# liupei101/AdvMIL

Measured on AMD Instinct MI355X. Metric: WSI bags/sec (full G+D step), higher is better.
Workload: dtype bf16x3 (fp32 operands split hi+lo, 3 bf16 MFMAs per product, fp32 accumulate; fp32 storage); 1 GPU; ABMIL+AdvMIL(RLIP prj discriminator), 8192-patch x 1024 fp32 bags (BASELINE.json configs[1] shape; fp32 storage, bf16x3 split arithmetic: >= the bf16 the config names, within 2e-5 of the fp32 reference); gen_updates=1, distinct_resident_bags_per_gpu=64, parallelism=bag-parallel dp1, dropout=shipped rates, launch=hipGraph replay (4 captured bag groups)

## Files before the change

### advmil_amd/_lib.py

```python
import ctypes
import os
from ctypes import c_float, c_int, c_int32, c_int64, c_size_t, c_uint64, c_void_p

LIB_PATH = os.environ.get("ADVMIL_HIP_LIB") or os.path.join(os.path.dirname(os.path.abspath(__file__)), "libadvmil_hip.so")


class HipLibraryMissing(RuntimeError):
    pass


class AdvmilHipError(RuntimeError):
    pass


class Epilogue(ctypes.Structure):
    _fields_ = [("bias", c_void_p), ("act0", c_int), ("act1", c_int), ("act_split", c_int), ("drop_p", c_float),
                ("seed", c_void_p), ("stream_id", c_uint64), ("rowv", c_void_p), ("colv", c_void_p), ("rowseg", c_void_p),
                ("maskref", c_void_p), ("ldmask", c_int), ("mask_scale", c_float), ("accumulate", c_int),
                ("alpha", c_float), ("a_hi", c_void_p), ("a_lo", c_void_p), ("b_hi", c_void_p), ("b_lo", c_void_p),
                ("c_hi", c_void_p), ("c_lo", c_void_p), ("gate_wc", c_void_p), ("gate_out", c_void_p), ("gate_np", c_int),
                ("rng_row", c_void_p), ("c2", c_void_p), ("ldc2", c_int64), ("n_split", c_int64), ("bias2", c_void_p), ("colsum", c_void_p), ("maskbits", c_void_p), ("ldbits", c_int64),
                ("gate_bits_a", c_void_p), ("gate_bits_b", c_void_p), ("ldgbits", c_int64), ("c_rows_pair32", c_int)]


# ... 35 lines not shown
                ("step", c_void_p), ("la_state", c_void_p), ("m_sched", c_void_p), ("p_hi", c_void_p), ("p_lo", c_void_p),
                ("abs_partial", c_void_p), ("clear_grad", ctypes.c_int32)]


OPT_KINDS = {"adam": 0, "adamw": 1, "nadam": 2, "radam": 3, "adadelta": 4}


SIGNATURES = {
    "advmil_version": (c_int, []),
    "advmil_gemm_f32_workspace_bytes": (c_size_t, [c_int64, c_int64, c_int]),
    "advmil_gemm_f32": (c_int, [c_int, c_int, c_int64, c_int64, c_int64, c_void_p, c_int64, c_void_p, c_int64, c_void_p,
                                c_int64, ctypes.POINTER(Epilogue), c_int, c_void_p, c_size_t, c_void_p]),
    "advmil_split_planes": (c_int, [c_void_p, c_int64, c_void_p, c_void_p, c_void_p]),
    "advmil_stage_bag": (c_int, [c_void_p, c_void_p, c_size_t, c_void_p, c_void_p, c_void_p, c_void_p, c_size_t, c_void_p]),
    "advmil_gate_interleave": (c_int, [c_void_p, c_void_p, c_void_p, c_void_p, c_int, c_void_p, c_void_p, c_void_p, c_void_p, c_int, c_void_p]),
    "advmil_gate_partial_sum": (c_int, [c_void_p, c_int, c_void_p, c_int64, c_void_p, c_void_p]),
    "advmil_gemm_f32_gate_blocks": (c_int, [c_int, c_int64]),
    "advmil_gemm_f32_colsum_rows": (c_int64, [c_int, c_int64, c_int64]),
    "advmil_merge_partials": (c_int, [c_void_p, c_int, c_int64, c_int64, c_void_p, c_int, c_void_p]),
    "advmil_set_gemm_mode": (c_int, [c_int]),
    "advmil_get_gemm_mode": (c_int, []),
    "advmil_gemm_f32_plan": (c_int, [c_int64, c_int64, c_int64, ctypes.POINTER(c_int), ctypes.POINTER(c_int)]),
    "advmil_gemm_f32_plan_layout": (c_int, [c_int, c_int, c_int64, c_int64, c_int64, ctypes.POINTER(c_int), ctypes.POINTER(c_int)]),
    "advmil_gemm_f32_plan_planes": (c_int, [c_int, c_int, c_int64, c_int64, c_int64, ctypes.POINTER(c_int)]),
    "advmil_gemm_f32_plan_tn_planes": (c_int, [c_int64, c_int64, c_int64, ctypes.POINTER(c_int), ctypes.POINTER(c_int)]),
    "advmil_gemm_f32_tiled": (c_int, [c_int, c_int, c_int64, c_int64, c_int64, c_void_p, c_int64, c_void_p, c_int64, c_void_p,
                                      c_int64, ctypes.POINTER(Epilogue), c_int, c_int, c_void_p, c_size_t, c_void_p]),
    "advmil_mha_fwd": (c_int, [c_void_p, c_void_p, c_int64, c_int, c_int, c_int, c_void_p, c_int64, c_float, c_void_p, c_uint64,
                               c_void_p, c_void_p, c_void_p, c_void_p]),
    "advmil_mha_fwd_lse": (c_int, [c_void_p, c_void_p, c_int64, c_int, c_int, c_int, c_void_p, c_int64, c_float, c_void_p, c_uint64,
# ... 10 lines not shown
    "advmil_add_dropout_ln_bwd": (c_int, [c_void_p, c_void_p, c_void_p, c_void_p, c_void_p, c_int64, c_int64, c_float, c_void_p,
                                          c_uint64, c_void_p, c_void_p, c_void_p, c_void_p, c_void_p, c_int, c_void_p, c_size_t,
                                          c_void_p]),
    "advmil_gate_score_fwd": (c_int, [c_void_p, c_void_p, c_void_p, c_float, c_void_p, c_uint64, c_uint64, c_int64, c_int64,
                                      c_void_p, c_void_p, c_void_p]),
    "advmil_softmax_pool_workspace_bytes": (c_size_t, [c_int64, c_int64, c_int]),
    "advmil_softmax_pool_fwd": (c_int, [c_void_p, c_void_p, c_int64, c_int64, c_int64, c_int, c_void_p, c_int64, c_void_p,
                                        c_void_p, c_void_p, c_size_t, c_void_p]),
    "advmil_softmax_pool_mean_workspace_bytes": (c_size_t, [c_int64, c_int64, c_int]),
    "advmil_softmax_pool_mean_fwd": (c_int, [c_void_p, c_void_p, c_int64, c_int64, c_int64, c_int, c_void_p, c_int64, c_void_p,
                                             c_void_p, c_void_p, c_void_p, c_size_t, c_void_p]),
    "advmil_softmax_pool_bwd": (c_int, [c_void_p, c_void_p, c_void_p, c_void_p, c_int64, c_int64, c_int64, c_int, c_void_p,
                                        c_int64, c_void_p, c_void_p, c_size_t, c_void_p]),
    "advmil_softmax_pool_fwd_planes": (c_int, [c_void_p, c_void_p, c_void_p, c_int64, c_int64, c_int64, c_int, c_void_p, c_int64, c_void_p,
                                               c_void_p, c_void_p, c_size_t, c_void_p]),
    "advmil_softmax_pool_bwd_planes": (c_int, [c_void_p, c_void_p, c_void_p, c_void_p, c_void_p, c_int64, c_int64, c_int64, c_int, c_void_p,
                                               c_int64, c_void_p, c_void_p, c_size_t, c_void_p]),
    "advmil_dropout_planes": (c_int, [c_void_p, c_void_p, c_int64, c_int64, c_float, c_void_p, c_uint64, c_void_p, c_void_p, c_void_p, c_void_p,
                                      c_float, c_uint64, c_uint64, c_void_p, c_void_p, c_void_p]),
    "advmil_gate_bwd_workspace_bytes": (c_size_t, [c_int64, c_int64]),
    "advmil_gate_bwd": (c_int, [c_void_p, c_void_p, c_void_p, c_float, c_void_p, c_uint64, c_uint64, c_int64, c_int64,
                                c_void_p, c_void_p, c_void_p, c_void_p, c_int, c_void_p, c_void_p, c_void_p, c_int, c_void_p, c_size_t,
                                c_void_p]),
    "advmil_colsum_workspace_bytes": (c_size_t, [c_int64, c_int64]),
    "advmil_act_dropout_bwd": (c_int, [c_void_p, c_void_p, c_int, c_float, c_void_p, c_uint64, c_int64, c_int64, c_void_p,
                                       c_void_p, c_int, c_void_p, c_void_p, c_void_p, c_void_p, c_void_p, c_size_t, c_void_p]),
    "advmil_colsum": (c_int, [c_void_p, c_int64, c_int64, c_void_p, c_int, c_void_p, c_size_t, c_void_p]),
    "advmil_ln_relu_mean16_fwd": (c_int, [c_void_p, c_void_p, c_void_p, c_float, c_int64, c_int64, c_void_p, c_void_p,
                                          c_void_p, c_void_p, c_void_p, c_int, c_void_p]),
    "advmil_ln_relu_mean16_bwd_workspace_bytes": (c_size_t, [c_int64, c_int64]),
# ... 102 lines not shown
```

### advmil_amd/csrc/pool.hip

```cpp
#include <cstdlib>
#include "common.h"
#include "bf16split.h"
#include "sumq.h"
#include "../../include/advmil_hip.h"

#define ROWS_PER_BLOCK 32
static inline int rows_per_block(int64_t rows) {
  int64_t r = (rows + 1023) / 1024;
  r = (r + 31) / 32 * 32;
  if (r < ROWS_PER_BLOCK) r = ROWS_PER_BLOCK;
  if (r > 512) r = 512;
  return (int)r;
}

struct RowColMap {
  int cols4, rpp, c4, r;
  bool active;
};
__device__ __forceinline__ RowColMap make_map(int64_t D) {
  RowColMap m;
  m.cols4 = (int)(D >> 2);
  m.rpp = 256 / m.cols4;
  if (m.rpp < 1) m.rpp = 1;
  m.c4 = threadIdx.x % m.cols4;
// ... 279 lines not shown
}

__device__ __forceinline__ void planes8(const bf16raw* __restrict__ hi, const bf16raw* __restrict__ lo, int64_t off, float4& v0, float4& v1) {
  const uint4 a = *reinterpret_cast<const uint4*>(hi + off);
  const uint4 b = *reinterpret_cast<const uint4*>(lo + off);
  v0.x = __uint_as_float(a.x << 16) + __uint_as_float(b.x << 16);
  v0.y = __uint_as_float(a.x & 0xffff0000u) + __uint_as_float(b.x & 0xffff0000u);
  v0.z = __uint_as_float(a.y << 16) + __uint_as_float(b.y << 16);
  v0.w = __uint_as_float(a.y & 0xffff0000u) + __uint_as_float(b.y & 0xffff0000u);
  v1.x = __uint_as_float(a.z << 16) + __uint_as_float(b.z << 16);
  v1.y = __uint_as_float(a.z & 0xffff0000u) + __uint_as_float(b.z & 0xffff0000u);
  v1.z = __uint_as_float(a.w << 16) + __uint_as_float(b.w << 16);
  v1.w = __uint_as_float(a.w & 0xffff0000u) + __uint_as_float(b.w & 0xffff0000u);
}

template <bool MEAN, bool PL = false>
__global__ __launch_bounds__(256) void pool_partial8_online_kernel(const float* __restrict__ s, const float* __restrict__ h, int64_t ldh,
                                                                   int64_t N, int64_t D, const int64_t* __restrict__ seg_ptr,
                                                                   float* __restrict__ partial, float* __restrict__ pstats, int rpb,
                                                                   float* __restrict__ mpartial, const bf16raw* __restrict__ hlo = nullptr) {
  __shared__ __attribute__((aligned(16))) float red[2048];
  __shared__ float wts[512];
  __shared__ float wred[8];
  const int cols8 = (int)(D >> 3), rpp = 256 / cols8;
  const int c8 = threadIdx.x % cols8, rl = threadIdx.x / cols8;
  const int tid = threadIdx.x, lane = tid & 63, w = tid >> 6;
  const int b = blockIdx.y;
  int64_t beg, end;
  seg_range(seg_ptr, b, N, beg, end);
  const int64_t r0 = beg + (int64_t)blockIdx.x * rpb;
  float* pst = pstats + ((int64_t)b * gridDim.x + blockIdx.x) * 2;
  float* prow = partial + ((int64_t)b * gridDim.x + blockIdx.x) * D;
  float* mrow = MEAN ? mpartial + ((int64_t)b * gridDim.x + blockIdx.x) * D : nullptr;
  if (r0 >= end) {
    if (tid < (int)(D >> 2)) {
      *reinterpret_cast<float4*>(prow + tid * 4) = make_float4(0.f, 0.f, 0.f, 0.f);
      if (MEAN) *reinterpret_cast<float4*>(mrow + tid * 4) = make_float4(0.f, 0.f, 0.f, 0.f);
    }
    if (tid == 0) { pst[0] = -INFINITY; pst[1] = 0.f; }
    return;
  }
  float mx = -INFINITY;
  for (int r = tid; r < rpb; r += 256) {
    const int64_t n = r0 + r;
    const float v = n < end ? s[n] : -INFINITY;
    wts[r] = v;
    mx = fmaxf(mx, v);
  }
  mx = wave_max(mx);
  if (lane == 0) wred[w] = mx;
  __syncthreads();
  mx = fmaxf(fmaxf(wred[0], wred[1]), fmaxf(wred[2], wred[3]));
  float ls = 0.f;
  for (int r = tid; r < rpb; r += 256) {
    const float e = (r0 + r < end) ? hw_exp(wts[r] - mx) : 0.f;
    wts[r] = e;
    ls += e;
  }
  ls = wave_sum(ls);
  if (lane == 0) wred[4 + w] = ls;
// ... 130 lines not shown
  }
  for (int64_t n = beg + (int64_t)blockIdx.x * 256 + tid; n < end; n += (int64_t)gridDim.x * 256) A[n] = hw_exp(s[n] - M) * inv;
}

static inline int64_t pool_nblk(int64_t max_len) { const int r = rows_per_block(max_len); return (max_len + r - 1) / r; }

extern "C" size_t advmil_softmax_pool_workspace_bytes(int64_t max_len, int64_t D, int nseg) {
  if (nseg < 1) nseg = 1;
  const int64_t a = 4 * (int64_t)nseg + (int64_t)nseg * pool_nblk(max_len) * (D + 2);
  const int64_t b = 4 + (int64_t)nseg * ((max_len + 3) / 4);
  return (size_t)(a > b ? a : b) * sizeof(float);
}

static int softmax_pool_fwd_impl(const float* s, const float* h, int64_t ldh, int64_t N, int64_t D, int nseg, const int64_t* seg_ptr,
                                 int64_t max_len, float* A, float* pooled, float* mean, void* ws, size_t ws_bytes, hipStream_t stream,
                                 const bf16raw* hlo = nullptr);

extern "C" int advmil_softmax_pool_fwd(const float* s, const float* h, int64_t ldh, int64_t N, int64_t D, int nseg,
                                       const int64_t* seg_ptr, int64_t max_len, float* A, float* pooled, void* ws,
                                       size_t ws_bytes, advmil_stream_t stream_) {
  return softmax_pool_fwd_impl(s, h, ldh, N, D, nseg, seg_ptr, max_len, A, pooled, nullptr, ws, ws_bytes, (hipStream_t)stream_);
}

extern "C" int advmil_softmax_pool_fwd_planes(const float* s, const void* h_hi, const void* h_lo, int64_t ldh, int64_t N, int64_t D, int nseg,
                                              const int64_t* seg_ptr, int64_t max_len, float* A, float* pooled, void* ws,
                                              size_t ws_bytes, advmil_stream_t stream_) {
  if (!h_hi || !h_lo) return ADVMIL_EINVAL;
  return softmax_pool_fwd_impl(s, (const float*)h_hi, ldh, N, D, nseg, seg_ptr, max_len, A, pooled, nullptr, ws, ws_bytes, (hipStream_t)stream_,
                               (const bf16raw*)h_lo);
}

static inline size_t pool_mean_offset_bytes(int64_t max_len, int64_t D, int nseg) {
  return (advmil_softmax_pool_workspace_bytes(max_len, D, nseg) + 15) / 16 * 16;
}

extern "C" size_t advmil_softmax_pool_mean_workspace_bytes(int64_t max_len, int64_t D, int nseg) {
  if (nseg < 1) nseg = 1;
  return pool_mean_offset_bytes(max_len, D, nseg) + (size_t)((int64_t)nseg * pool_nblk(max_len) * D) * sizeof(float);
}

extern "C" int advmil_softmax_pool_mean_fwd(const float* s, const float* h, int64_t ldh, int64_t N, int64_t D, int nseg,
                                            const int64_t* seg_ptr, int64_t max_len, float* A, float* pooled, float* mean, void* ws,
                                            size_t ws_bytes, advmil_stream_t stream_) {
  if (!mean) return ADVMIL_EINVAL;
  return softmax_pool_fwd_impl(s, h, ldh, N, D, nseg, seg_ptr, max_len, A, pooled, mean, ws, ws_bytes, (hipStream_t)stream_);
}

static int softmax_pool_fwd_impl(const float* s, const float* h, int64_t ldh, int64_t N, int64_t D, int nseg, const int64_t* seg_ptr,
                                 int64_t max_len, float* A, float* pooled, float* mean, void* ws, size_t ws_bytes, hipStream_t stream,
                                 const bf16raw* hlo) {
  if (!s || !h || !A || !pooled || !ws || N <= 0 || D <= 0 || (D & 3) || D > 1024 || (ldh & 3)) return ADVMIL_EINVAL;
  if (ldh < D || ((uintptr_t)h & 15)) return ADVMIL_EINVAL;
  if (hlo && (((uintptr_t)hlo & 15) || (D & 7) || (ldh & 7) || D < 16 || mean)) return ADVMIL_EINVAL;
  if (!seg_ptr && nseg > 1) return ADVMIL_EINVAL;
  if (!seg_ptr) { nseg = 1; max_len = N; }
  if (nseg < 1 || max_len <= 0 || max_len > N) return ADVMIL_EINVAL;
  if (ws_bytes < (mean ? advmil_softmax_pool_mean_workspace_bytes(max_len, D, nseg) : advmil_softmax_pool_workspace_bytes(max_len, D, nseg)))
    return ADVMIL_EWORKSPACE;
  float* stats = (float*)ws;
  float* partial = stats + 4 * nseg;
  const int nblk = (int)pool_nblk(max_len);
  if ((D & 7) == 0 && D >= 16 && nblk <= POOL_ONLINE_MAX_NBLK) {
    float* pstats = partial + (int64_t)nseg * nblk * D;
    if (mean) {
      float* mpartial = (float*)ws + pool_mean_offset_bytes(max_len, D, nseg) / sizeof(float);
      hipLaunchKernelGGL((pool_partial8_online_kernel<true, false>), dim3(nblk, nseg), dim3(256), 0, stream, s, h, ldh, N, D, seg_ptr, partial, pstats,
                         rows_per_block(max_len), mpartial, (const bf16raw*)nullptr);
      ADVMIL_LAUNCH_CHECK();
      hipLaunchKernelGGL(pool_merge_online_kernel, dim3((unsigned)((D + 15) / 16), nseg), dim3(256), 0, stream, partial, pstats, nblk, D, s,
                         N, seg_ptr, pooled, A, stats, (const float*)mpartial, mean);
      ADVMIL_LAUNCH_CHECK();
      return ADVMIL_OK;
    }
    if (hlo)
      hipLaunchKernelGGL((pool_partial8_online_kernel<false, true>), dim3(nblk, nseg), dim3(256), 0, stream, s, h, ldh, N, D, seg_ptr, partial,
                         pstats, rows_per_block(max_len), (float*)nullptr, hlo);
    else
      hipLaunchKernelGGL((pool_partial8_online_kernel<false, false>), dim3(nblk, nseg), dim3(256), 0, stream, s, h, ldh, N, D, seg_ptr, partial,
                         pstats, rows_per_block(max_len), (float*)nullptr, (const bf16raw*)nullptr);
    ADVMIL_LAUNCH_CHECK();
    hipLaunchKernelGGL(pool_merge_online_kernel, dim3((unsigned)((D + 15) / 16), nseg), dim3(256), 0, stream, partial, pstats, nblk, D, s,
                       N, seg_ptr, pooled, A, stats, (const float*)nullptr, (float*)nullptr);
    ADVMIL_LAUNCH_CHECK();
    return ADVMIL_OK;
  }
  if (mean || hlo) return ADVMIL_EINVAL;
  hipLaunchKernelGGL(softmax_stats_kernel, dim3(nseg), dim3(1024), 0, stream, s, N, seg_ptr, stats);
  ADVMIL_LAUNCH_CHECK();
  if ((D & 7) == 0 && D >= 16)
    hipLaunchKernelGGL(pool_partial8_kernel, dim3(nblk, nseg), dim3(256), 0, stream, s, h, ldh, N, D, seg_ptr, stats, A, partial,
                       rows_per_block(max_len));
  else
    hipLaunchKernelGGL(pool_partial_kernel, dim3(nblk, nseg), dim3(256), 0, stream, s, h, ldh, N, D, seg_ptr, stats, A, partial,
                       rows_per_block(max_len));
  ADVMIL_LAUNCH_CHECK();
  hipLaunchKernelGGL(colsum_merge_kernel, dim3((unsigned)((D + 15) / 16), nseg), dim3(256), 0, stream, partial, nblk, D, D, pooled,
                     0, (int64_t)nblk * D, D);
  ADVMIL_LAUNCH_CHECK();
  return ADVMIL_OK;
}

// ... 232 lines not shown
  for (int64_t n = (int64_t)blockIdx.x * 256 + threadIdx.x; n < N; n += (int64_t)gridDim.x * 256) {
    float a = 0.f;
    for (int j = 0; j < np; ++j) a += partial[n * np + j];
    s[n] = a + b;
  }
}
extern "C" int advmil_gate_interleave(const float* Wa, const float* Wb, const float* ba, const float* bb, int D, float* Wi, void* Wi_hi,
                                      void* Wi_lo, float* bi, int pair32, advmil_stream_t stream_) {
  if (!Wa || !Wb || !ba || !bb || !Wi || !bi || D <= 0 || (D & 3) || ((Wi_hi != nullptr) != (Wi_lo != nullptr))) return ADVMIL_EINVAL;
  if (pair32 && (D & 31)) return ADVMIL_EINVAL;
  if (((uintptr_t)Wa & 15) || ((uintptr_t)Wb & 15) || ((uintptr_t)Wi & 15) || ((uintptr_t)Wi_hi & 7) || ((uintptr_t)Wi_lo & 7)) return ADVMIL_EINVAL;
  int64_t blocks = ((int64_t)2 * D * (D >> 2) + 255) / 256;
  if (blocks > 1024) blocks = 1024;
  hipLaunchKernelGGL(gate_interleave_kernel, dim3((unsigned)blocks), dim3(256), 0, (hipStream_t)stream_, Wa, Wb, ba, bb, D, Wi,
                     (bf16raw*)Wi_hi, (bf16raw*)Wi_lo, bi, pair32);
  ADVMIL_LAUNCH_CHECK();
  return ADVMIL_OK;
}
extern "C" int advmil_gate_partial_sum(const float* partial, int np, const float* bc, int64_t N, float* s, advmil_stream_t stream_) {
  if (!partial || !s || np <= 0 || N <= 0) return ADVMIL_EINVAL;
  int64_t blocks = (N + 255) / 256;
  if (blocks > 2048) blocks = 2048;
  hipLaunchKernelGGL(gate_partial_sum_kernel, dim3((unsigned)blocks), dim3(256), 0, (hipStream_t)stream_, partial, np, bc, N, s);
  ADVMIL_LAUNCH_CHECK();
  return ADVMIL_OK;
}

__global__ __launch_bounds__(256) void gate_bwd_kernel(const float* __restrict__ ab, const float* __restrict__ ds,
                                                       const float* __restrict__ wc, float p, const uint64_t* seed,
                                                       uint64_t stream_a, uint64_t stream_b, int64_t N, int64_t D,
// ... 839 lines not shown
```

### advmil_amd/ops.py

```python
import ctypes
import os

import torch

from . import _lib
from ._lib import Epilogue

ACT_NONE, ACT_RELU, ACT_TANH, ACT_SIGMOID = 0, 1, 2, 3
FUSED_WGRAD = True
KERNEL_PROFILE = None
STAMPS = None


class Stamps:

    def __init__(self, device, cap=2048):
        self.buf = torch.zeros(cap, dtype=torch.int64, device=device)
        self.tags = []
        self.khz = int(_lib.lib().advmil_clock_rate_khz()) or 100000

    def mark(self, tag):
        i = len(self.tags)
        if i >= self.buf.numel():
            return
# ... 296 lines not shown
        return Planes(torch.empty_strided(x.shape, x.stride(), dtype=torch.bfloat16, device=x.device),
                      torch.empty_strided(x.shape, x.stride(), dtype=torch.bfloat16, device=x.device))

    def view_rows(self, r0, r1):
        return Planes(self.hi[r0:r1], None if self.lo is None else self.lo[r0:r1])


USE_PLANES = os.environ.get("ADVMIL_PLANES", "1") != "0"
DH_NT_FUSED = os.environ.get("ADVMIL_DH_NT_FUSED", "1") != "0"
ACT_BWD_IN_DH = os.environ.get("ADVMIL_ACT_BWD_IN_DH", "1") != "0"
DG_PLANES_ONLY = os.environ.get("ADVMIL_DG_PLANES_ONLY", "1") != "0"
DW_PLANES = os.environ.get("ADVMIL_DW_PLANES", "1") != "0"
MEMO_PLANES = os.environ.get("ADVMIL_MEMO_PLANES", "1") != "0"
H_PLANES_ONLY = os.environ.get("ADVMIL_H_PLANES_ONLY", "1") != "0"
FUSED_GATE_TRAIN = os.environ.get("ADVMIL_FUSED_GATE_TRAIN", "1") != "0"
SLAB_PLANES_ANY = os.environ.get("ADVMIL_SLAB_PLANES_ANY", "1") != "0"
GENERIC_PLANES = os.environ.get("ADVMIL_GENERIC_PLANES", "1") != "0"
SMALL_LINEAR = os.environ.get("ADVMIL_SMALL_LINEAR", "1") != "0"
SMALL_LINEAR_ROWS = int(os.environ.get("ADVMIL_SMALL_LINEAR_ROWS", "8"))


def slab_takes_planes(rows, C):
    return bool(rows >= 4096 and USE_PLANES and get_gemm_mode() == "bf16x3" and (SLAB_PLANES_ANY or gemm_plan_planes(rows, 128, C)))


def planes_transposed(pl):
    R, C = pl.hi.shape
    out = Planes.alloc((C, R), pl.hi.device)
    d = (pl.lo.data_ptr() - pl.hi.data_ptr()) // 2
    do = (out.lo.data_ptr() - out.hi.data_ptr()) // 2
# ... 320 lines not shown
            self._div[k] = Segments([v // k for v in self.lens], self.device)
        return self._div[k]

    def twice(self):
        if "x2" not in self._div:
            self._div["x2"] = Segments(self.lens + self.lens, self.device)
        return self._div["x2"]

    def uniform(self, rows):
        key = ("u", rows)
        if key not in self._div:
            self._div[key] = Segments([rows] * self.nseg, self.device)
        return self._div[key]


def softmax_pool(s, h, N, D, seg=None, hpl=None):
    L = _lib.lib()
    nseg = 1 if seg is None else seg.nseg
    mlen = N if seg is None else seg.max_len
    A = torch.empty(N, dtype=torch.float32, device=h.device)
    pooled = torch.empty(nseg, D, dtype=torch.float32, device=h.device)
    wsb = L.advmil_softmax_pool_workspace_bytes(mlen, D, nseg)
    ws = _ws(wsb, h.device)
    big = STAMPS is not None and N * D >= (1 << 24)
    if big:
        _stamp("b", "softmax_pool_fwd", (N, D, nseg), 4.0 * N * D + 12.0 * N)
    if hpl is not None:
        _lib.check(L.advmil_softmax_pool_fwd_planes(_p(s), _p(hpl.hi), _p(hpl.lo), hpl.hi.stride(0), N, D, nseg,
                                                    _p(None if seg is None else seg.ptr), mlen, _p(A), _p(pooled), _p(ws), wsb, _stream()),
                   "softmax_pool_fwd_planes")
    else:
        _lib.check(L.advmil_softmax_pool_fwd(_p(s), _p(h), h.stride(0), N, D, nseg, _p(None if seg is None else seg.ptr), mlen, _p(A),
                                             _p(pooled), _p(ws), wsb, _stream()), "softmax_pool_fwd")
    if big:
        _stamp("e", "softmax_pool_fwd", (N, D, nseg), 4.0 * N * D + 12.0 * N)
    return A, pooled


def softmax_pool_mean(s, h, N, D, seg=None):
    L = _lib.lib()
    nseg = 1 if seg is None else seg.nseg
    mlen = N if seg is None else seg.max_len
    A = torch.empty(N, dtype=torch.float32, device=h.device)
    pooled = torch.empty(nseg, D, dtype=torch.float32, device=h.device)
    mean = torch.empty(nseg, D, dtype=torch.float32, device=h.device)
    wsb = L.advmil_softmax_pool_mean_workspace_bytes(mlen, D, nseg)
    ws = _ws(wsb, h.device)
    _lib.check(L.advmil_softmax_pool_mean_fwd(_p(s), _p(h), h.stride(0), N, D, nseg, _p(None if seg is None else seg.ptr), mlen, _p(A),
                                              _p(pooled), _p(mean), _p(ws), wsb, _stream()), "softmax_pool_mean_fwd")
    return A, pooled, mean

# ... 384 lines not shown
            if xpl is None and is_bf16_slab(x):
                x = as_f32(x)
            if ctx.gW is not None:
                gemm(dpre, x, False, False, N, K, M, out=ctx.gW.view(N, K), ldc=K, accumulate=True, b_planes=xpl)
            else:
                dW = gemm(dpre, x, False, False, N, K, M, b_planes=xpl).reshape(wshape)
        dx = gemm(dpre, W2, True, False, M, K, N) if need_x else None
        return dx, dW, (None if ctx.gb is not None else db), None, None, None, None, None, None, None, None, None


class ForwardMemo:

    def __init__(self):
        self.mode, self.token, self.rows_ptr, self.store = None, None, None, {}
        self.derived, self.ln = {}, {}

    def begin(self, mode, token, rows):
        if token != self.token:
            self.store.clear(); self.derived.clear(); self.ln.clear()
        self.mode, self.token, self.rows_ptr = mode, token, rows.data_ptr()

    def knows(self, x):
        return self.mode is not None and (x.data_ptr() == self.rows_ptr or (MEMO_CHAIN and x.data_ptr() in self.derived))

    def end(self, clear=False):
        self.mode = None
        if clear:
            self.store.clear(); self.derived.clear(); self.ln.clear()


MEMO = ForwardMemo()
MEMO_CHAIN = os.environ.get("ADVMIL_MEMO_CHAIN", "1") != "0"
MEMO_MIN_ROWS = int(os.environ.get("ADVMIL_MEMO_MIN_ROWS", "4096"))


PREFILL = {}
TWO_LAYERS = os.environ.get("ADVMIL_TWO_LAYERS", "1") != "0"


def prefill_two_layers(X, layer1, layer2):
    (W1, b1, a1, emit1), (W2, b2, a2, _) = layer1, layer2
    if not TWO_LAYERS or X.dim() != 2 or not X.is_contiguous():
        return False
# ... 101 lines not shown


class GatedAttnPoolFn(torch.autograd.Function):

    @staticmethod
    def forward(ctx, h, Wa, ba, Wb, bb, wc, bc, p, seed, sa, sb, seg, nograd=False, rr=None, hpl=None, act_fuse=None, gate=None):
        _chk(h, "h")
        h = h.contiguous()
        N, D = h.shape
        ctx.act_fuse = act_fuse
        ctx.pair32 = False
        wcv = wc.detach().reshape(-1)
        stale = hpl is not None and hpl.fp32_stale
        ppl = hpl if stale else None
        if FUSED_GATE_SCORE and p <= 0.0 and N >= 4096 and nograd:
            Wi, bi, wipl = gate_interleave(Wa.detach(), ba.detach(), Wb.detach(), bb.detach(), D, planes=hpl is not None)
            s = gate_partial_sum(gemm(h, Wi, True, True, N, 2 * D, D, bias=bi, gate_wc=wcv, a_planes=hpl, b_planes=wipl), bc.detach())
            A, pooled = softmax_pool(s, h, N, D, seg, ppl)
            ctx.mark_non_differentiable(s)
            return pooled, A, s
        gs = [_arena_grad(t) for t in (Wa, ba, Wb, bb, wc, bc)]
        arena_ok = all(g is not None for g in gs) and _adjacent(gs[0], gs[2]) and _adjacent(gs[1], gs[3])
        if (gate is not None and FUSED_GATE_TRAIN and p > 0.0 and hpl is not None and arena_ok and N % 256 == 0 and D % 64 == 0
                and get_gemm_mode() == "bf16x3" and gemm_plan_planes(N, 2 * D, D) and gemm_plan_tn_planes(2 * D, D, N)[1] > 1
                and gemm_plan_planes(N, D, 2 * D)):
            Wp, bp, wppl = gate_interleave(Wa.detach(), ba.detach(), Wb.detach(), bb.detach(), D, planes=True, pair32=True)
            ab, part = gemm(h, Wp, True, True, N, 2 * D, D, bias=bp, gate_wc=wcv, drop_p=p, a_planes=hpl, b_planes=wppl, gate_bits=gate)
            s = gate_partial_sum(part, bc.detach())
            A, pooled = softmax_pool(s, h, N, D, seg, ppl)
            ctx.save_for_backward(h, Wp, ab, A, wcv)
            ctx.hpl, ctx.wabpl, ctx.pair32 = hpl, wppl, True
            ctx.cfg = (p, seed, sa, sb, N, D, wc.shape, seg, rr)
            ctx.arena = (gs[0].as_strided((2 * D, D), (D, 1), gs[0].storage_offset()),
                         gs[1].as_strided((2 * D,), (1,), gs[1].storage_offset()), gs[4].view(-1), gs[5])
            ctx.mark_non_differentiable(s)
            ctx.set_materialize_grads(False)
            return pooled, A, s
        Wab, _ = _stack2(Wa, Wb, D, D)
        bab, _ = _stack2(ba, bb, D, 0)
        wabpl = None
        if hpl is not None:
            pa_, pb_ = weight_planes(Wa), weight_planes(Wb)
            if pa_ is not None and pb_ is not None and _adjacent(pa_.hi, pb_.hi, 2) and _adjacent(pa_.lo, pb_.lo, 2):
                wabpl = Planes(pa_.hi.as_strided((2 * D, D), (D, 1), pa_.hi.storage_offset()),
# ... 39 lines not shown
            gpl = Planes.alloc((N, 2 * D), h.device)
        if ctx.arena is not None:
            gWab, gbab, gwc, gbc = ctx.arena
            dG, _, _, _ = gate_bwd(ab, ds, wcv, N, D, p, seed, sa, sb, dwc=gwc, dbc=gbc, dbias=gbab, rng_row=rr, planes=gpl, planes_only=only,
                                   pair32=pair32)
        else:
            dG, dwc, dbc, dbias = gate_bwd(ab, ds, wcv, N, D, p, seed, sa, sb, rng_row=rr, planes=gpl, planes_only=only)
        dh = None
        fuse = ctx.act_fuse if (need_h and only and ctx.act_fuse is not None) else None
        if fuse is not None and stale and fuse[2] is None:
            fuse = None
        wtpl = None
        if fuse is not None and dh_nt:
            nrow = int(_lib.lib().advmil_gemm_f32_colsum_rows(dh_tile, N, D))
            tile = dh_tile
            wtpl = planes_transposed(ctx.wabpl)
        elif fuse is not None:
            tile = gemm_plan(N, D, 2 * D, True, False)[0]
            nrow = int(_lib.lib().advmil_gemm_f32_colsum_rows(tile, N, D)) if pre_a_tile_ok(tile, True, False) else 0
            if nrow <= 0:
                fuse = None
        if fuse is not None:
            p1, gb1, mbits = fuse
            dpl = Planes.alloc((N, D), h.device)
            cws = _ws(nrow * D * 4, h.device) if gb1 is not None else None
            if wtpl is not None:
                gemm(None, None, True, True, N, D, 2 * D, rowv=A, colv=dpooled, rowseg=None if seg is None else seg.rowseg, a_planes=gpl,
                     b_planes=wtpl, maskbits=mbits, mask_scale=1.0 / (1.0 - p1) if p1 > 0.0 else 1.0, c_planes=dpl, c_planes_only=True,
                     colsum=cws, tile=tile)
            else:
                gemm(None, Wab, True, False, N, D, 2 * D, rowv=A, colv=dpooled, rowseg=None if seg is None else seg.rowseg, a_planes=gpl,
# ... 632 lines not shown


def skinny_linear(x, W, b, act="none"):
    return SkinnyLinearFn.apply(x, W, b, _ACT[act])


def gate_interleave(Wa, ba, Wb, bb, D, planes=False, pair32=False):
    Wa, Wb, ba, bb = (t.contiguous() for t in (Wa, Wb, ba, bb))
    dev = Wa.device
    Wi = torch.empty(2 * D, D, dtype=torch.float32, device=dev)
    bi = torch.empty(2 * D, dtype=torch.float32, device=dev)
    pl = Planes.alloc((2 * D, D), dev) if planes else None
    _lib.check(_lib.lib().advmil_gate_interleave(_p(Wa), _p(Wb), _p(ba), _p(bb), D, _p(Wi), _p(None if pl is None else pl.hi),
                                                 _p(None if pl is None else pl.lo), _p(bi), 1 if pair32 else 0, _stream()), "gate_interleave")
    return Wi, bi, pl


def gate_partial_sum(partial, bc=None):
    partial = partial.contiguous()
    N, npart = partial.shape
    s = torch.empty(N, dtype=torch.float32, device=partial.device)
    _lib.check(_lib.lib().advmil_gate_partial_sum(_p(partial), npart, _p(None if bc is None else bc.reshape(-1)), N, _p(s), _stream()),
               "gate_partial_sum")
    return s


class PrjHeadFn(torch.autograd.Function):

    @staticmethod
    def forward(ctx, u, t, src, W, b):
# ... 383 lines not shown
```

### include/advmil_hip.h

```cpp
#ifndef ADVMIL_HIP_H
#define ADVMIL_HIP_H
#include <stddef.h>
#include <stdint.h>

#ifdef __cplusplus
extern "C" {
#endif

typedef void* advmil_stream_t;

enum { ADVMIL_ACT_NONE = 0, ADVMIL_ACT_RELU = 1, ADVMIL_ACT_TANH = 2, ADVMIL_ACT_SIGMOID = 3 };

int advmil_version(void);

typedef struct {
  const float* bias;
  int act0, act1, act_split;
  float drop_p;
  const uint64_t* seed;
  uint64_t stream_id;
  const float* rowv;
  const float* colv;
  const int32_t* rowseg;
  const float* maskref;
// ... 19 lines not shown
  const uint32_t* maskbits;
  int64_t ldbits;
  const uint32_t* gate_bits_a;
  const uint32_t* gate_bits_b;
  int64_t ldgbits;
  int c_rows_pair32;
} advmil_epilogue_t;

size_t advmil_gemm_f32_workspace_bytes(int64_t M, int64_t N, int splits);
int advmil_gemm_f32(int a_kc, int b_kc, int64_t M, int64_t N, int64_t K, const float* A, int64_t lda,
                    const float* B, int64_t ldb, float* C, int64_t ldc, const advmil_epilogue_t* epi,
                    int splits, void* ws, size_t ws_bytes, advmil_stream_t stream);
int advmil_split_planes(const float* src, int64_t n, void* hi, void* lo, advmil_stream_t stream);
int advmil_gate_interleave(const float* Wa, const float* Wb, const float* ba, const float* bb, int D, float* Wi, void* Wi_hi, void* Wi_lo,
                           float* bi, int pair32, advmil_stream_t stream);
int advmil_gate_partial_sum(const float* partial, int np, const float* bc, int64_t N, float* s, advmil_stream_t stream);
int advmil_gemm_f32_gate_blocks(int tile, int64_t N);
int64_t advmil_gemm_f32_colsum_rows(int tile, int64_t M, int64_t N);
int advmil_merge_partials(const float* partial, int nblk, int64_t stride, int64_t ncols, float* out, int accumulate, advmil_stream_t stream);
int advmil_set_gemm_mode(int mode);
int advmil_get_gemm_mode(void);
int advmil_gemm_f32_plan(int64_t M, int64_t N, int64_t K, int* tile, int* splits);
int advmil_gemm_f32_plan_layout(int a_kc, int b_kc, int64_t M, int64_t N, int64_t K, int* tile, int* splits);
int advmil_gemm_f32_plan_planes(int a_kc, int b_kc, int64_t M, int64_t N, int64_t K, int* tile);
int advmil_gemm_f32_plan_tn_planes(int64_t M, int64_t N, int64_t K, int* tile, int* splits);
int advmil_gemm_f32_tiled(int a_kc, int b_kc, int64_t M, int64_t N, int64_t K, const float* A, int64_t lda,
                          const float* B, int64_t ldb, float* C, int64_t ldc, const advmil_epilogue_t* epi,
                          int splits, int tile, void* ws, size_t ws_bytes, advmil_stream_t stream);

int advmil_mha_fwd(const void* qkv_hi, const void* qkv_lo, int64_t Ltot, int nhead, int head_dim, int nseg, const int64_t* ptr,
// ... 23 lines not shown
                          uint64_t stream_a, uint64_t stream_b, int64_t N, int64_t D, float* s, const int64_t* rng_row,
                          advmil_stream_t stream);
size_t advmil_softmax_pool_workspace_bytes(int64_t max_len, int64_t D, int nseg);
int advmil_softmax_pool_fwd(const float* s, const float* h, int64_t ldh, int64_t N, int64_t D, int nseg,
                            const int64_t* seg_ptr, int64_t max_len, float* A, float* pooled, void* ws, size_t ws_bytes,
                            advmil_stream_t stream);
size_t advmil_softmax_pool_mean_workspace_bytes(int64_t max_len, int64_t D, int nseg);
int advmil_softmax_pool_mean_fwd(const float* s, const float* h, int64_t ldh, int64_t N, int64_t D, int nseg, const int64_t* seg_ptr,
                                 int64_t max_len, float* A, float* pooled, float* mean, void* ws, size_t ws_bytes, advmil_stream_t stream);
int advmil_softmax_pool_bwd(const float* dpooled, const float* dA, const float* A, const float* h, int64_t ldh,
                            int64_t N, int64_t D, int nseg, const int64_t* seg_ptr, int64_t max_len, float* ds, void* ws,
                            size_t ws_bytes, advmil_stream_t stream);
int advmil_softmax_pool_fwd_planes(const float* s, const void* h_hi, const void* h_lo, int64_t ldh, int64_t N, int64_t D, int nseg,
                                   const int64_t* seg_ptr, int64_t max_len, float* A, float* pooled, void* ws, size_t ws_bytes,
                                   advmil_stream_t stream);
int advmil_softmax_pool_bwd_planes(const float* dpooled, const float* dA, const float* A, const void* h_hi, const void* h_lo, int64_t ldh,
                                   int64_t N, int64_t D, int nseg, const int64_t* seg_ptr, int64_t max_len, float* ds, void* ws,
                                   size_t ws_bytes, advmil_stream_t stream);
int advmil_dropout_planes(const void* in_hi, const void* in_lo, int64_t M, int64_t N, float drop_p, const uint64_t* seed, uint64_t stream_id,
                          const int64_t* rng_row, void* out_hi, void* out_lo, void* bits, float gate_p, uint64_t gate_stream_a,
                          uint64_t gate_stream_b, void* gate_bits_a, void* gate_bits_b, advmil_stream_t stream);
int advmil_seg_scale_rows(const float* dpooled, const float* A, const int32_t* rowseg, int64_t N, int64_t D, float* dh,
                          advmil_stream_t stream);
size_t advmil_gate_bwd_workspace_bytes(int64_t N, int64_t D);
int advmil_gate_bwd(const float* ab, const float* ds, const float* wc, float drop_p, const uint64_t* seed,
                    uint64_t stream_a, uint64_t stream_b, int64_t N, int64_t D, float* dG, float* dwc, float* dbc,
                    float* dbias, int accumulate, const int64_t* rng_row, void* dG_hi, void* dG_lo, int pair32, void* ws, size_t ws_bytes,
                    advmil_stream_t stream);

size_t advmil_colsum_workspace_bytes(int64_t M, int64_t N);
// ... 212 lines not shown
```

Before: 5843 bags/s.

## Fuse gate partial-sum into softmax pool and build all gate weight operands once

```diff
diff --git a/advmil_amd/_lib.py b/advmil_amd/_lib.py
--- a/advmil_amd/_lib.py
+++ b/advmil_amd/_lib.py
@@ -73,6 +73,8 @@
     "advmil_split_planes": (c_int, [c_void_p, c_int64, c_void_p, c_void_p, c_void_p]),
     "advmil_stage_bag": (c_int, [c_void_p, c_void_p, c_size_t, c_void_p, c_void_p, c_void_p, c_void_p, c_size_t, c_void_p]),
     "advmil_gate_interleave": (c_int, [c_void_p, c_void_p, c_void_p, c_void_p, c_int, c_void_p, c_void_p, c_void_p, c_void_p, c_int, c_void_p]),
+    "advmil_gate_operands": (c_int, [c_void_p, c_void_p, c_void_p, c_void_p, c_int, c_void_p, c_void_p, c_void_p, c_void_p, c_void_p, c_void_p,
+                                     c_void_p, c_void_p, c_void_p, c_void_p, c_void_p]),
     "advmil_gate_partial_sum": (c_int, [c_void_p, c_int, c_void_p, c_int64, c_void_p, c_void_p]),
     "advmil_gemm_f32_gate_blocks": (c_int, [c_int, c_int64]),
     "advmil_gemm_f32_colsum_rows": (c_int64, [c_int, c_int64, c_int64]),
@@ -113,6 +115,8 @@
                                         c_int64, c_void_p, c_void_p, c_size_t, c_void_p]),
     "advmil_softmax_pool_fwd_planes": (c_int, [c_void_p, c_void_p, c_void_p, c_int64, c_int64, c_int64, c_int, c_void_p, c_int64, c_void_p,
                                                c_void_p, c_void_p, c_size_t, c_void_p]),
+    "advmil_softmax_pool_fwd_parts": (c_int, [c_void_p, c_int, c_void_p, c_void_p, c_void_p, c_void_p, c_int64, c_int64, c_int64, c_int, c_void_p,
+                                              c_int64, c_void_p, c_void_p, c_void_p, c_size_t, c_void_p]),
     "advmil_softmax_pool_bwd_planes": (c_int, [c_void_p, c_void_p, c_void_p, c_void_p, c_void_p, c_int64, c_int64, c_int64, c_int, c_void_p,
                                                c_int64, c_void_p, c_void_p, c_size_t, c_void_p]),
     "advmil_dropout_planes": (c_int, [c_void_p, c_void_p, c_int64, c_int64, c_float, c_void_p, c_uint64, c_void_p, c_void_p, c_void_p, c_void_p,
diff --git a/advmil_amd/csrc/pool.hip b/advmil_amd/csrc/pool.hip
--- a/advmil_amd/csrc/pool.hip
+++ b/advmil_amd/csrc/pool.hip
@@ -317,11 +317,13 @@
   v1.w = __uint_as_float(a.w & 0xffff0000u) + __uint_as_float(b.w & 0xffff0000u);
 }
 
-template <bool MEAN, bool PL = false>
+template <bool MEAN, bool PL = false, bool PARTS = false>
 __global__ __launch_bounds__(256) void pool_partial8_online_kernel(const float* __restrict__ s, const float* __restrict__ h, int64_t ldh,
                                                                    int64_t N, int64_t D, const int64_t* __restrict__ seg_ptr,
                                                                    float* __restrict__ partial, float* __restrict__ pstats, int rpb,
-                                                                   float* __restrict__ mpartial, const bf16raw* __restrict__ hlo = nullptr) {
+                                                                   float* __restrict__ mpartial, const bf16raw* __restrict__ hlo = nullptr,
+                                                                   int np = 0, const float* __restrict__ bc = nullptr,
+                                                                   float* __restrict__ s_out = nullptr) {
   __shared__ __attribute__((aligned(16))) float red[2048];
   __shared__ float wts[512];
   __shared__ float wred[8];
@@ -344,9 +346,20 @@
     return;
   }
   float mx = -INFINITY;
+  const float bcv = (PARTS && bc) ? bc[0] : 0.f;
   for (int r = tid; r < rpb; r += 256) {
     const int64_t n = r0 + r;
-    const float v = n < end ? s[n] : -INFINITY;
+    float v = -INFINITY;
+    if constexpr (PARTS) {
+      if (n < end) {
+        float a = 0.f;
+        for (int j = 0; j < np; ++j) a += s[n * np + j];
+        v = a + bcv;
+        s_out[n] = v;
+      }
+    } else {
+      v = n < end ? s[n] : -INFINITY;
+    }
     wts[r] = v;
     mx = fmaxf(mx, v);
   }
@@ -507,7 +520,7 @@
 
 static int softmax_pool_fwd_impl(const float* s, const float* h, int64_t ldh, int64_t N, int64_t D, int nseg, const int64_t* seg_ptr,
                                  int64_t max_len, float* A, float* pooled, float* mean, void* ws, size_t ws_bytes, hipStream_t stream,
-                                 const bf16raw* hlo = nullptr);
+                                 const bf16raw* hlo = nullptr, const float* parts = nullptr, int np = 0, const float* bc = nullptr);
 
 extern "C" int advmil_softmax_pool_fwd(const float* s, const float* h, int64_t ldh, int64_t N, int64_t D, int nseg,
                                        const int64_t* seg_ptr, int64_t max_len, float* A, float* pooled, void* ws,
@@ -523,6 +536,14 @@
                                (const bf16raw*)h_lo);
 }
 
+extern "C" int advmil_softmax_pool_fwd_parts(const float* parts, int np, const float* bc, float* s, const void* h, const void* h_lo,
+                                             int64_t ldh, int64_t N, int64_t D, int nseg, const int64_t* seg_ptr, int64_t max_len, float* A,
+                                             float* pooled, void* ws, size_t ws_bytes, advmil_stream_t stream_) {
+  if (!parts || np <= 0) return ADVMIL_EINVAL;
+  return softmax_pool_fwd_impl(s, (const float*)h, ldh, N, D, nseg, seg_ptr, max_len, A, pooled, nullptr, ws, ws_bytes, (hipStream_t)stream_,
+                               (const bf16raw*)h_lo, parts, np, bc);
+}
+
 static inline size_t pool_mean_offset_bytes(int64_t max_len, int64_t D, int nseg) {
   return (advmil_softmax_pool_workspace_bytes(max_len, D, nseg) + 15) / 16 * 16;
 }
@@ -541,7 +562,8 @@
 
 static int softmax_pool_fwd_impl(const float* s, const float* h, int64_t ldh, int64_t N, int64_t D, int nseg, const int64_t* seg_ptr,
                                  int64_t max_len, float* A, float* pooled, float* mean, void* ws, size_t ws_bytes, hipStream_t stream,
-                                 const bf16raw* hlo) {
+                                 const bf16raw* hlo, const float* parts, int np, const float* bc) {
+  if (parts && (np <= 0 || mean)) return ADVMIL_EINVAL;
   if (!s || !h || !A || !pooled || !ws || N <= 0 || D <= 0 || (D & 3) || D > 1024 || (ldh & 3)) return ADVMIL_EINVAL;
   if (ldh < D || ((uintptr_t)h & 15)) return ADVMIL_EINVAL;
   if (hlo && (((uintptr_t)hlo & 15) || (D & 7) || (ldh & 7) || D < 16 || mean)) return ADVMIL_EINVAL;
@@ -565,7 +587,13 @@
       ADVMIL_LAUNCH_CHECK();
       return ADVMIL_OK;
     }
-    if (hlo)
+    if (parts && hlo)
+      hipLaunchKernelGGL((pool_partial8_online_kernel<false, true, true>), dim3(nblk, nseg), dim3(256), 0, stream, parts, h, ldh, N, D, seg_ptr,
+                         partial, pstats, rows_per_block(max_len), (float*)nullptr, hlo, np, bc, (float*)s);
+    else if (parts)
+      hipLaunchKernelGGL((pool_partial8_online_kernel<false, false, true>), dim3(nblk, nseg), dim3(256), 0, stream, parts, h, ldh, N, D, seg_ptr,
+                         partial, pstats, rows_per_block(max_len), (float*)nullptr, (const bf16raw*)nullptr, np, bc, (float*)s);
+    else if (hlo)
       hipLaunchKernelGGL((pool_partial8_online_kernel<false, true>), dim3(nblk, nseg), dim3(256), 0, stream, s, h, ldh, N, D, seg_ptr, partial,
                          pstats, rows_per_block(max_len), (float*)nullptr, hlo);
     else
@@ -577,7 +605,7 @@
     ADVMIL_LAUNCH_CHECK();
     return ADVMIL_OK;
   }
-  if (mean || hlo) return ADVMIL_EINVAL;
+  if (mean || hlo || parts) return ADVMIL_EINVAL;
   hipLaunchKernelGGL(softmax_stats_kernel, dim3(nseg), dim3(1024), 0, stream, s, N, seg_ptr, stats);
   ADVMIL_LAUNCH_CHECK();
   if ((D & 7) == 0 && D >= 16)
@@ -840,6 +868,64 @@
   if (blocks > 1024) blocks = 1024;
   hipLaunchKernelGGL(gate_interleave_kernel, dim3((unsigned)blocks), dim3(256), 0, (hipStream_t)stream_, Wa, Wb, ba, bb, D, Wi,
                      (bf16raw*)Wi_hi, (bf16raw*)Wi_lo, bi, pair32);
+  ADVMIL_LAUNCH_CHECK();
+  return ADVMIL_OK;
+}
+__global__ __launch_bounds__(256) void gate_operands_kernel(const float* __restrict__ Wa, const float* __restrict__ Wb,
+                                                            const float* __restrict__ ba, const float* __restrict__ bb, int D,
+                                                            float* __restrict__ Wi, bf16raw* __restrict__ ihi, bf16raw* __restrict__ ilo,
+                                                            float* __restrict__ bi, float* __restrict__ Wp, bf16raw* __restrict__ phi,
+                                                            bf16raw* __restrict__ plo, float* __restrict__ bp, bf16raw* __restrict__ thi,
+                                                            bf16raw* __restrict__ tlo) {
+  const int q4 = D >> 2, R = 2 * D;
+  const int64_t total = (int64_t)R * q4;
+  for (int64_t e = (int64_t)blockIdx.x * 256 + threadIdx.x; e < total; e += (int64_t)gridDim.x * 256) {
+    const int r = (int)(e / q4), c = (int)(e % q4) * 4;
+    uint2 hh, ll;
+    {
+      const float4 v = *reinterpret_cast<const float4*>(((r & 1) ? Wb : Wa) + (int64_t)(r >> 1) * D + c);
+      *reinterpret_cast<float4*>(Wi + (int64_t)r * D + c) = v;
+      split4(v, hh, ll);
+      *reinterpret_cast<uint2*>(ihi + (int64_t)r * D + c) = hh;
+      *reinterpret_cast<uint2*>(ilo + (int64_t)r * D + c) = ll;
+    }
+    {
+      const float4 v = *reinterpret_cast<const float4*>((((r >> 5) & 1) ? Wb : Wa) + (int64_t)(((r >> 6) << 5) | (r & 31)) * D + c);
+      *reinterpret_cast<float4*>(Wp + (int64_t)r * D + c) = v;
+      split4(v, hh, ll);
+      *reinterpret_cast<uint2*>(phi + (int64_t)r * D + c) = hh;
+      *reinterpret_cast<uint2*>(plo + (int64_t)r * D + c) = ll;
+    }
+  }
+  for (int64_t e = (int64_t)blockIdx.x * 256 + threadIdx.x; e < total; e += (int64_t)gridDim.x * 256) {
+    const int r = (int)(e % R), c = (int)(e / R) * 4;
+    const float4 v = *reinterpret_cast<const float4*>((((r >> 5) & 1) ? Wb : Wa) + (int64_t)(((r >> 6) << 5) | (r & 31)) * D + c);
+    uint2 hh, ll;
+    split4(v, hh, ll);
+    thi[(int64_t)c * R + r] = (bf16raw)(hh.x & 0xffffu);       tlo[(int64_t)c * R + r] = (bf16raw)(ll.x & 0xffffu);
+    thi[(int64_t)(c + 1) * R + r] = (bf16raw)(hh.x >> 16);     tlo[(int64_t)(c + 1) * R + r] = (bf16raw)(ll.x >> 16);
+    thi[(int64_t)(c + 2) * R + r] = (bf16raw)(hh.y & 0xffffu); tlo[(int64_t)(c + 2) * R + r] = (bf16raw)(ll.y & 0xffffu);
+    thi[(int64_t)(c + 3) * R + r] = (bf16raw)(hh.y >> 16);     tlo[(int64_t)(c + 3) * R + r] = (bf16raw)(ll.y >> 16);
+  }
+  if (blockIdx.x == 0)
+    for (int r = threadIdx.x; r < R; r += 256) {
+      bi[r] = (r & 1) ? bb[r >> 1] : ba[r >> 1];
+      const int j = ((r >> 6) << 5) | (r & 31);
+      bp[r] = ((r >> 5) & 1) ? bb[j] : ba[j];
+    }
+}
+extern "C" int advmil_gate_operands(const float* Wa, const float* Wb, const float* ba, const float* bb, int D, float* Wi, void* Wi_hi, void* Wi_lo,
+                                    float* bi, float* Wp, void* Wp_hi, void* Wp_lo, float* bp, void* WpT_hi, void* WpT_lo,
+                                    advmil_stream_t stream_) {
+  if (!Wa || !Wb || !ba || !bb || !Wi || !Wi_hi || !Wi_lo || !bi || !Wp || !Wp_hi || !Wp_lo || !bp || !WpT_hi || !WpT_lo || D <= 0 || (D & 31))
+    return ADVMIL_EINVAL;
+  if ((((uintptr_t)Wa | (uintptr_t)Wb | (uintptr_t)Wi | (uintptr_t)Wp) & 15) ||
+      (((uintptr_t)Wi_hi | (uintptr_t)Wi_lo | (uintptr_t)Wp_hi | (uintptr_t)Wp_lo) & 7) || (((uintptr_t)WpT_hi | (uintptr_t)WpT_lo) & 1))
+    return ADVMIL_EINVAL;
+  int64_t blocks = ((int64_t)2 * D * (D >> 2) + 255) / 256;
+  if (blocks > 1024) blocks = 1024;
+  hipLaunchKernelGGL(gate_operands_kernel, dim3((unsigned)blocks), dim3(256), 0, (hipStream_t)stream_, Wa, Wb, ba, bb, D, Wi, (bf16raw*)Wi_hi,
+                     (bf16raw*)Wi_lo, bi, Wp, (bf16raw*)Wp_hi, (bf16raw*)Wp_lo, bp, (bf16raw*)WpT_hi, (bf16raw*)WpT_lo);
   ADVMIL_LAUNCH_CHECK();
   return ADVMIL_OK;
 }
diff --git a/advmil_amd/ops.py b/advmil_amd/ops.py
--- a/advmil_amd/ops.py
+++ b/advmil_amd/ops.py
@@ -334,6 +334,8 @@
 MEMO_PLANES = os.environ.get("ADVMIL_MEMO_PLANES", "1") != "0"
 H_PLANES_ONLY = os.environ.get("ADVMIL_H_PLANES_ONLY", "1") != "0"
 FUSED_GATE_TRAIN = os.environ.get("ADVMIL_FUSED_GATE_TRAIN", "1") != "0"
+POOL_SUMS_PARTS = os.environ.get("ADVMIL_POOL_SUMS_PARTS", "1") != "0"
+GATE_OPERANDS = os.environ.get("ADVMIL_GATE_OPERANDS", "1") != "0"
 SLAB_PLANES_ANY = os.environ.get("ADVMIL_SLAB_PLANES_ANY", "1") != "0"
 GENERIC_PLANES = os.environ.get("ADVMIL_GENERIC_PLANES", "1") != "0"
 SMALL_LINEAR = os.environ.get("ADVMIL_SMALL_LINEAR", "1") != "0"
@@ -684,7 +686,11 @@
         return self._div[key]
 
 
-def softmax_pool(s, h, N, D, seg=None, hpl=None):
+def pool_takes_parts(mlen, D):
+    return D % 8 == 0 and D >= 16 and mlen <= 2048 * 512
+
+
+def softmax_pool(s, h, N, D, seg=None, hpl=None, parts=None, bc=None):
     L = _lib.lib()
     nseg = 1 if seg is None else seg.nseg
     mlen = N if seg is None else seg.max_len
@@ -695,7 +701,15 @@
     big = STAMPS is not None and N * D >= (1 << 24)
     if big:
         _stamp("b", "softmax_pool_fwd", (N, D, nseg), 4.0 * N * D + 12.0 * N)
-    if hpl is not None:
+    if parts is not None:
+        parts = parts.contiguous()
+        s = torch.empty(N, dtype=torch.float32, device=h.device)
+        src = h if hpl is None else hpl.hi
+        _lib.check(L.advmil_softmax_pool_fwd_parts(_p(parts), parts.shape[1], _p(None if bc is None else bc.reshape(-1)), _p(s), _p(src),
+                                                   _p(None if hpl is None else hpl.lo), src.stride(0), N, D, nseg,
+                                                   _p(None if seg is None else seg.ptr), mlen, _p(A), _p(pooled), _p(ws), wsb, _stream()),
+                   "softmax_pool_fwd_parts")
+    elif hpl is not None:
         _lib.check(L.advmil_softmax_pool_fwd_planes(_p(s), _p(hpl.hi), _p(hpl.lo), hpl.hi.stride(0), N, D, nseg,
                                                     _p(None if seg is None else seg.ptr), mlen, _p(A), _p(pooled), _p(ws), wsb, _stream()),
                    "softmax_pool_fwd_planes")
@@ -704,7 +718,16 @@
                                              _p(pooled), _p(ws), wsb, _stream()), "softmax_pool_fwd")
     if big:
         _stamp("e", "softmax_pool_fwd", (N, D, nseg), 4.0 * N * D + 12.0 * N)
-    return A, pooled
+    return (A, pooled, s) if parts is not None else (A, pooled)
+
+
+def gate_parts_pool(part, bc, h, N, D, seg, hpl):
+    if POOL_SUMS_PARTS and pool_takes_parts(N if seg is None else seg.max_len, D):
+        A, pooled, s = softmax_pool(None, h, N, D, seg, hpl, parts=part, bc=bc)
+    else:
+        s = gate_partial_sum(part, bc)
+        A, pooled = softmax_pool(s, h, N, D, seg, hpl)
+    return s, A, pooled
 
 
 def softmax_pool_mean(s, h, N, D, seg=None):
@@ -1119,10 +1142,11 @@
     def __init__(self):
         self.mode, self.token, self.rows_ptr, self.store = None, None, None, {}
         self.derived, self.ln = {}, {}
+        self.gate = {}
 
     def begin(self, mode, token, rows):
         if token != self.token:
-            self.store.clear(); self.derived.clear(); self.ln.clear()
+            self.store.clear(); self.derived.clear(); self.ln.clear(); self.gate.clear()
         self.mode, self.token, self.rows_ptr = mode, token, rows.data_ptr()
 
     def knows(self, x):
@@ -1131,7 +1155,7 @@
     def end(self, clear=False):
         self.mode = None
         if clear:
-            self.store.clear(); self.derived.clear(); self.ln.clear()
+            self.store.clear(); self.derived.clear(); self.ln.clear(); self.gate.clear()
 
 
 MEMO = ForwardMemo()
@@ -1263,9 +1287,13 @@
         stale = hpl is not None and hpl.fp32_stale
         ppl = hpl if stale else None
         if FUSED_GATE_SCORE and p <= 0.0 and N >= 4096 and nograd:
-            Wi, bi, wipl = gate_interleave(Wa.detach(), ba.detach(), Wb.detach(), bb.detach(), D, planes=hpl is not None)
-            s = gate_partial_sum(gemm(h, Wi, True, True, N, 2 * D, D, bias=bi, gate_wc=wcv, a_planes=hpl, b_planes=wipl), bc.detach())
-            A, pooled = softmax_pool(s, h, N, D, seg, ppl)
+            if GATE_OPERANDS and D % 32 == 0:
+                Wi, bi, wipl = gate_operands_for(Wa, ba, Wb, bb, D)[:3]
+                wipl = wipl if hpl is not None else None
+            else:
+                Wi, bi, wipl = gate_interleave(Wa.detach(), ba.detach(), Wb.detach(), bb.detach(), D, planes=hpl is not None)
+            part = gemm(h, Wi, True, True, N, 2 * D, D, bias=bi, gate_wc=wcv, a_planes=hpl, b_planes=wipl)
+            s, A, pooled = gate_parts_pool(part, bc.detach(), h, N, D, seg, ppl)
             ctx.mark_non_differentiable(s)
             return pooled, A, s
         gs = [_arena_grad(t) for t in (Wa, ba, Wb, bb, wc, bc)]
@@ -1273,10 +1301,13 @@
         if (gate is not None and FUSED_GATE_TRAIN and p > 0.0 and hpl is not None and arena_ok and N % 256 == 0 and D % 64 == 0
                 and get_gemm_mode() == "bf16x3" and gemm_plan_planes(N, 2 * D, D) and gemm_plan_tn_planes(2 * D, D, N)[1] > 1
                 and gemm_plan_planes(N, D, 2 * D)):
-            Wp, bp, wppl = gate_interleave(Wa.detach(), ba.detach(), Wb.detach(), bb.detach(), D, planes=True, pair32=True)
+            ctx.wtpl = None
+            if GATE_OPERANDS:
+                Wp, bp, wppl, ctx.wtpl = gate_operands_for(Wa, ba, Wb, bb, D)[3:]
+            else:
+                Wp, bp, wppl = gate_interleave(Wa.detach(), ba.detach(), Wb.detach(), bb.detach(), D, planes=True, pair32=True)
             ab, part = gemm(h, Wp, True, True, N, 2 * D, D, bias=bp, gate_wc=wcv, drop_p=p, a_planes=hpl, b_planes=wppl, gate_bits=gate)
-            s = gate_partial_sum(part, bc.detach())
-            A, pooled = softmax_pool(s, h, N, D, seg, ppl)
+            s, A, pooled = gate_parts_pool(part, bc.detach(), h, N, D, seg, ppl)
             ctx.save_for_backward(h, Wp, ab, A, wcv)
             ctx.hpl, ctx.wabpl, ctx.pair32 = hpl, wppl, True
             ctx.cfg = (p, seed, sa, sb, N, D, wc.shape, seg, rr)
@@ -1346,7 +1377,9 @@
         if fuse is not None and dh_nt:
             nrow = int(_lib.lib().advmil_gemm_f32_colsum_rows(dh_tile, N, D))
             tile = dh_tile
-            wtpl = planes_transposed(ctx.wabpl)
+            wtpl = getattr(ctx, "wtpl", None)
+            if wtpl is None:
+                wtpl = planes_transposed(ctx.wabpl)
         elif fuse is not None:
             tile = gemm_plan(N, D, 2 * D, True, False)[0]
             nrow = int(_lib.lib().advmil_gemm_f32_colsum_rows(tile, N, D)) if pre_a_tile_ok(tile, True, False) else 0
@@ -2009,6 +2042,32 @@
     _lib.check(_lib.lib().advmil_gate_interleave(_p(Wa), _p(Wb), _p(ba), _p(bb), D, _p(Wi), _p(None if pl is None else pl.hi),
                                                  _p(None if pl is None else pl.lo), _p(bi), 1 if pair32 else 0, _stream()), "gate_interleave")
     return Wi, bi, pl
+
+
+def gate_operands(Wa, ba, Wb, bb, D):
+    Wa, Wb, ba, bb = (t.contiguous() for t in (Wa, Wb, ba, bb))
+    dev = Wa.device
+    Wi, Wp = torch.empty(2 * D, D, dtype=torch.float32, device=dev), torch.empty(2 * D, D, dtype=torch.float32, device=dev)
+    bi, bp = torch.empty(2 * D, dtype=torch.float32, device=dev), torch.empty(2 * D, dtype=torch.float32, device=dev)
+    ipl, ppl, tpl = Planes.alloc((2 * D, D), dev), Planes.alloc((2 * D, D), dev), Planes.alloc((D, 2 * D), dev)
+    _lib.check(_lib.lib().advmil_gate_operands(_p(Wa), _p(Wb), _p(ba), _p(bb), D, _p(Wi), _p(ipl.hi), _p(ipl.lo), _p(bi), _p(Wp), _p(ppl.hi),
+                                               _p(ppl.lo), _p(bp), _p(tpl.hi), _p(tpl.lo), _stream()), "gate_operands")
+    return Wi, bi, ipl, Wp, bp, ppl, tpl
+
+
+def gate_operands_for(Wa, ba, Wb, bb, D):
+    key = tuple((t.data_ptr(), t._version) for t in (Wa, ba, Wb, bb)) + (D,)
+    if MEMO.mode == "replay":
+        ent = MEMO.gate.pop(key, None)
+        if ent is not None:
+            for t in ent:
+                for u in ((t.hi, t.lo) if isinstance(t, Planes) else (t,)):
+                    u.record_stream(torch.cuda.current_stream())
+            return ent
+    ent = gate_operands(Wa.detach(), ba.detach(), Wb.detach(), bb.detach(), D)
+    if MEMO.mode == "record":
+        MEMO.gate[key] = ent
+    return ent
 
 
 def gate_partial_sum(partial, bc=None):
diff --git a/include/advmil_hip.h b/include/advmil_hip.h
--- a/include/advmil_hip.h
+++ b/include/advmil_hip.h
@@ -57,6 +57,8 @@
 int advmil_split_planes(const float* src, int64_t n, void* hi, void* lo, advmil_stream_t stream);
 int advmil_gate_interleave(const float* Wa, const float* Wb, const float* ba, const float* bb, int D, float* Wi, void* Wi_hi, void* Wi_lo,
                            float* bi, int pair32, advmil_stream_t stream);
+int advmil_gate_operands(const float* Wa, const float* Wb, const float* ba, const float* bb, int D, float* Wi, void* Wi_hi, void* Wi_lo,
+                         float* bi, float* Wp, void* Wp_hi, void* Wp_lo, float* bp, void* WpT_hi, void* WpT_lo, advmil_stream_t stream);
 int advmil_gate_partial_sum(const float* partial, int np, const float* bc, int64_t N, float* s, advmil_stream_t stream);
 int advmil_gemm_f32_gate_blocks(int tile, int64_t N);
 int64_t advmil_gemm_f32_colsum_rows(int tile, int64_t M, int64_t N);
@@ -110,6 +112,9 @@
 int advmil_softmax_pool_fwd_planes(const float* s, const void* h_hi, const void* h_lo, int64_t ldh, int64_t N, int64_t D, int nseg,
                                    const int64_t* seg_ptr, int64_t max_len, float* A, float* pooled, void* ws, size_t ws_bytes,
                                    advmil_stream_t stream);
+int advmil_softmax_pool_fwd_parts(const float* parts, int np, const float* bc, float* s, const void* h, const void* h_lo, int64_t ldh,
+                                  int64_t N, int64_t D, int nseg, const int64_t* seg_ptr, int64_t max_len, float* A, float* pooled, void* ws,
+                                  size_t ws_bytes, advmil_stream_t stream);
 int advmil_softmax_pool_bwd_planes(const float* dpooled, const float* dA, const float* A, const void* h_hi, const void* h_lo, int64_t ldh,
                                    int64_t N, int64_t D, int nseg, const int64_t* seg_ptr, int64_t max_len, float* ds, void* ws,
                                    size_t ws_bytes, advmil_stream_t stream);
```

Measured after the change: 5852 bags/s (median of 4 runs). About the same (+0.2%).
